# arjunchandra/paac

Hardware: AMD Instinct MI355X
Metric: global env-steps/sec at 32 envs, t_max=5, Nature net; 1/2/4/8 MI355X (higher is better)
Workload: dtype f32; 1 GPU; breakout action set (A=4), NATURE net, 32 envs per GPU x 1 GPU, t_max=5, synthetic 84x84x4 u8 frames generated on device, sampler=numpy, hipGraph replay; envs_per_gpu=32, t_max=5, global_envs=32, parallelism=env-sharded dp1, no collective (one process)

## Files before the change

paac_amd/csrc/api.hip:

```cpp
#include <stdarg.h>
#include <stdlib.h>

#include <new>

#include "common.h"

namespace paac {

static thread_local char g_err[512] = "";
thread_local ProfEvents g_prof = {nullptr, nullptr, 0, 0};
paac_ctx* g_prof_ctx = nullptr;

void set_error(const char* fmt, ...) {
  va_list ap;
  va_start(ap, fmt);
  vsnprintf(g_err, sizeof(g_err), fmt, ap);
  va_end(ap);
}

ArchSpec arch_spec(int arch) {
  ArchSpec s;
  memset(&s, 0, sizeof(s));
  if (arch == PAAC_ARCH_NATURE) {
    s.nconv = 3;
// ... 131 lines not shown
  c->max_batch = cfg->max_batch;
  for (int o = 0; o < OP_COUNT; ++o)
    for (int k = 0; k < 3; ++k) c->tune[o][k] = Tune{-1, 0, -1};
  default_tuning(c);
  if (const char* ov = getenv("PAAC_TUNE_OVERRIDE")) {
    int op, cls, cf, ks, xc, used = 0;
    while (sscanf(ov, "%d:%d:%d:%d:%d%n", &op, &cls, &cf, &ks, &xc, &used) == 5) {
      if (op >= 0 && op < OP_COUNT && cls >= 0 && cls < 3) c->tune[op][cls] = Tune{cf, ks, xc};
      ov += used;
      if (*ov != ',') break;
      ++ov;
    }
  }
  const int64_t B = cfg->max_batch;
  const int A = cfg->num_actions;
  c->fc_splits_max = fc_splits_max();
  for (int w = 0; w < 2; ++w) {
    Workspace& W = c->ws[w];
    for (int i = 0; i < c->spec.nconv; ++i) {
      const ConvSpec& cs = c->spec.conv[i];
      PAAC_CHECK_HIP(hipMalloc(&W.act[i], (size_t)((B + 15) / 16 * 16) * cs.oh * cs.ow * cs.cout * sizeof(float)));
    }
    PAAC_CHECK_HIP(hipMalloc(&W.fc_slab, (size_t)c->fc_splits_max * B * c->spec.fc * sizeof(float)));
    PAAC_CHECK_HIP(hipMalloc(&W.h, (size_t)B * c->spec.fc * sizeof(float)));
    PAAC_CHECK_HIP(hipMalloc(&W.probs, (size_t)B * A * sizeof(float)));
    PAAC_CHECK_HIP(hipMalloc(&W.logits, (size_t)B * A * sizeof(float)));
    PAAC_CHECK_HIP(hipMalloc(&W.values, (size_t)B * sizeof(float)));
  }
  for (int i = 0; i < c->spec.nconv; ++i) {
    const ConvSpec& cs = c->spec.conv[i];
    PAAC_CHECK_HIP(hipMalloc(&c->dact[i], (size_t)B * cs.oh * cs.ow * cs.cout * sizeof(float)));
  }
  PAAC_CHECK_HIP(hipMalloc(&c->dh, (size_t)B * c->spec.fc * sizeof(float)));
  PAAC_CHECK_HIP(hipMalloc(&c->dl_buf, (size_t)B * paac::kDlStride * sizeof(float)));
  PAAC_CHECK_HIP(hipMalloc(&c->ppo_rows, (size_t)B * 2 * sizeof(float)));
  PAAC_CHECK_HIP(hipMalloc(&c->vclip_rows, (size_t)B * sizeof(float)));
  c->wslab_floats = wslab_floats_needed(cfg->arch);
  PAAC_CHECK_HIP(hipMalloc(&c->wslab, (size_t)c->wslab_floats * sizeof(float)));
  PAAC_CHECK_HIP(hipMalloc(&c->partials, 8192 * sizeof(float)));
  PAAC_CHECK_HIP(hipMemset(c->partials, 0, 8192 * sizeof(float)));
  PAAC_CHECK_HIP(hipMalloc(&c->zeros, (size_t)(c->spec.fc > 1024 ? c->spec.fc : 1024) * sizeof(float)));
  PAAC_CHECK_HIP(hipMemset(c->zeros, 0, (size_t)(c->spec.fc > 1024 ? c->spec.fc : 1024) * sizeof(float)));
  c->keep_row = -1;
  c->keep_h_only = 0;
  c->heads_pending_h = 0;
  PAAC_CHECK_HIP(hipMalloc(&c->mt_ahead, mt_ahead_bytes()));
  PAAC_CHECK_HIP(hipMemset(c->mt_ahead, 0, mt_ahead_bytes()));
  c->ahead_state = nullptr;
  c->ahead_D = 0;
  {
    const char* v = getenv("PAAC_TOWER");
    c->tower_on = (cfg->arch == PAAC_ARCH_NATURE) && !(v && *v && atoi(v) == 0);
    { const char* q = getenv("PAAC_FC_QUARTER"); c->no_quarter_tiles = (q && *q && atoi(q) == 0) ? 1 : 0; }
    c->tower2_on = (cfg->arch == PAAC_ARCH_NIPS) && tower2_available() && !(v && *v && atoi(v) == 0);
    c->managed_weights = 0;
    c->tower_pack = nullptr;
    if (c->tower_on || c->tower2_on) PAAC_CHECK_HIP(hipMalloc(&c->tower_pack, tower_pack_bytes()));
    PAAC_CHECK_HIP(hipMalloc(&c->fc_pack, (size_t)c->spec.flat * c->spec.fc * sizeof(float)));
  }
  c->ev_start = new hipEvent_t[paac_ctx::PROF_MAX_EVENTS];
  c->ev_stop = new hipEvent_t[paac_ctx::PROF_MAX_EVENTS];
  c->ev_family = new int[paac_ctx::PROF_MAX_EVENTS];
  c->ev_batch = new int[paac_ctx::PROF_MAX_EVENTS];
  c->ev_mix = new int[paac_ctx::PROF_MAX_EVENTS];
  c->ev_count = 0;
  c->prof_on = 0;
  for (int i = 0; i < paac_ctx::PROF_MAX_EVENTS; ++i) {
    c->ev_start[i] = nullptr;
    c->ev_stop[i] = nullptr;
  }
  *out = c;
  return 0;
}

int paac_destroy(paac_ctx* c) {
  if (!c) return 0;
  for (int w = 0; w < 2; ++w) {
    Workspace& W = c->ws[w];
    for (int i = 0; i < 3; ++i)
      if (W.act[i]) (void)hipFree(W.act[i]);
    float* bufs[] = {W.fc_slab, W.h, W.probs, W.logits, W.values};
    for (float* b : bufs)
      if (b) (void)hipFree(b);
  }
  for (int i = 0; i < 3; ++i)
    if (c->dact[i]) (void)hipFree(c->dact[i]);
  float* bufs[] = {c->dh, c->wslab, c->partials, c->dl_buf, c->zeros, c->ppo_rows, c->vclip_rows};
  for (float* b : bufs)
    if (b) (void)hipFree(b);
  if (c->mt_ahead) (void)hipFree(c->mt_ahead);
  if (c->tower_pack) (void)hipFree(c->tower_pack);
  if (c->fc_pack) (void)hipFree(c->fc_pack);
  for (int i = 0; i < paac_ctx::PROF_MAX_EVENTS; ++i) {
    if (c->ev_start[i]) (void)hipEventDestroy(c->ev_start[i]);
    if (c->ev_stop[i]) (void)hipEventDestroy(c->ev_stop[i]);
  }
  delete[] c->ev_start;
  delete[] c->ev_stop;
  delete[] c->ev_family;
  delete[] c->ev_batch;
  delete[] c->ev_mix;
  delete c;
  return 0;
}

int paac_forward(paac_ctx* ctx, const float* params, const uint8_t* states, int batch, float* logits, float* probs,
                 float* values, paac_stream_t stream) {
  PAAC_REQUIRE(ctx && params && states, "paac_forward: null argument");
  PAAC_REQUIRE(batch > 0 && batch <= ctx->max_batch, "paac_forward: batch %d outside (0, max_batch=%d]", batch,
               ctx->max_batch);
  const int rc = launch_forward(ctx, 0, params, states, batch, logits, probs, values, (hipStream_t)stream);
  if (rc) return rc;
  PAAC_CHECK_HIP(hipGetLastError());
  return 0;
}

int paac_pack_weights(paac_ctx* ctx, const float* params, paac_stream_t stream) {
  PAAC_REQUIRE(ctx && params, "paac_pack_weights: null argument");
  const int rc = launch_pack_weights(ctx, params, (hipStream_t)stream);
  if (rc) return rc;
  PAAC_CHECK_HIP(hipGetLastError());
  return 0;
}
// ... 555 lines not shown
```

paac_amd/csrc/common.h:

```cpp
#pragma once
#include <hip/hip_runtime.h>
#include <hip/hip_ext.h>
#include <stdint.h>
#include <stdio.h>
#include <string.h>

#include "../../include/paac_hip.h"

namespace paac {

void set_error(const char* fmt, ...);

#define PAAC_CHECK_HIP(expr)                                                              \
  do {                                                                                    \
    hipError_t _e = (expr);                                                               \
    if (_e != hipSuccess) {                                                               \
      paac::set_error("%s:%d: %s -> %s", __FILE__, __LINE__, #expr, hipGetErrorString(_e)); \
      return -2;                                                                          \
    }                                                                                     \
  } while (0)

#define PAAC_REQUIRE(cond, ...)          \
  do {                                   \
    if (!(cond)) {                       \
// ... 19 lines not shown
enum Family {
  F_CONV1_FWD = 0, F_CONV2_FWD, F_CONV3_FWD, F_FC_FWD, F_HEADS_FWD,
  F_HEADS_BWD, F_FC_WGRAD, F_FC_DGRAD, F_CONV3_WGRAD, F_CONV3_DGRAD, F_CONV2_WGRAD, F_CONV2_DGRAD, F_CONV1_WGRAD,
  F_GRAD_FINALIZE, F_CLIP_RMSPROP, F_MISC,
  F_ENV_STEP, F_SAMPLE_ENV_STEP, F_SAMPLE_MT, F_SAMPLE_PHILOX, F_NSTEP_RETURNS, F_PREPROCESS_STACK, F_CONV_TOWER,
  F_FC_CONV3_WGRAD, F_CONV2_CONV1_WGRAD, F_DGRAD_TOWER
};
static_assert(F_DGRAD_TOWER + 1 == PAAC_PROF_FAMILIES, "family count");

}

namespace paac {
struct Workspace {
  float* act[3];
  float* fc_slab;
  float* h;
  float* probs;
  float* values;
  float* logits;
};
}

namespace paac {
enum Op { OP_CONV1_FWD = 0, OP_CONV2_FWD, OP_CONV3_FWD, OP_FC_FWD, OP_FC_WGRAD, OP_FC_DGRAD, OP_CONV3_WGRAD,
          OP_CONV3_DGRAD, OP_CONV2_WGRAD, OP_CONV2_DGRAD, OP_CONV1_WGRAD, OP_CONV_TOWER, OP_COUNT };
struct Tune {
  int cfg;
  int ksplit;
  int xcd;
};
inline int batch_class(int batch) { return batch > 512 ? 2 : batch > 64 ? 1 : 0; }

constexpr int kDlStride = 36;

struct FinalizeSeg {
  const float* src;
  float* dst;
  int count;
  int splits;
  long stride;
};
struct FinalizeArgs {
  FinalizeSeg seg[8];
  int nseg;
};

}

struct paac_ctx {
  paac_cfg cfg;
  paac::Tune tune[paac::OP_COUNT][3];
  paac::ArchSpec spec;
  paac_layout layout;
  int max_batch;
  paac::Workspace ws[2];
  int last_ws;
  float* dact[3];
  float* dh;
  float* wslab;
  int64_t wslab_floats;
  float* partials;
  int last_clip_local;
  paac::FinalizeArgs pending_fin;
  const float* pending_fin_grad;
  int heads_pending_rows, heads_pending_splits;
  int keep_row;
  int keep_h_only;
  int heads_pending_h;
  float* zeros;
  void* mt_ahead;
  const uint32_t* ahead_state;
  int ahead_D;
  float* dl_buf;
  float* ppo_rows;
  float* vclip_rows;
  int fc_splits_max;
  void* tower_pack;
  void* fc_pack;
  int tower_on;
  int heads_ntiles;
  int no_quarter_tiles;
  int tower2_on;
  int managed_weights;
  int prof_on;
  static constexpr int PROF_MAX_EVENTS = 8192;
  hipEvent_t* ev_start;
  hipEvent_t* ev_stop;
  int* ev_family;
  int* ev_batch;
  int* ev_mix;
  int ev_count;
// ... 106 lines not shown
```

paac_amd/csrc/heads.h:

```cpp
#pragma once
#include "common.h"
#include "synth_dev.h"

namespace paac {

constexpr int FC_SPLITS_MAX = 8;
constexpr int MAXA = 32;

#ifdef PAAC_DMM_STAMPS
__device__ unsigned long long* g_stamps_dev = nullptr;
#define HEADS_STAMP_INIT() unsigned long long* stamp_ptr = g_stamps_dev
#define HEADS_STAMP(i)                                                                                         \
  do {                                                                                                         \
    __builtin_amdgcn_sched_barrier(0);                                                                         \
    if (stamp_ptr && threadIdx.x == 0) stamp_ptr[(long)blockIdx.x * 8 + (i)] = (unsigned long long)clock64(); \
    __builtin_amdgcn_sched_barrier(0);                                                                         \
  } while (0)
#else
#define HEADS_STAMP_INIT()
#define HEADS_STAMP(i)
#endif

template <int NV>
__device__ __forceinline__ void block_sums_256(const float (&vals)[NV], float* scratch, float* out_lds) {
  const int tid = threadIdx.x;
#pragma unroll
  for (int a = 0; a < NV; ++a) scratch[a * 256 + tid] = vals[a];
  __syncthreads();
  float* stage = scratch + NV * 256;
  for (int u = tid; u < NV * 8; u += 256) {
    const int a = u >> 3, c = u & 7;
    float v[32];
#pragma unroll
    for (int i = 0; i < 32; ++i) v[i] = scratch[a * 256 + c * 32 + ((i + c) & 31)];
// ... 409 lines not shown
    ceps = rt.ppo.clip_eps;
  }
  if constexpr (LOSS == kLossPpoVclip) {
    vold = rt.vc.v_old[i];
    veps = rt.vc.vclip_eps;
  }
  if (rt.v_boot) {
    returns_row(rt, i, yv, av);
  } else {
    yv = y[i];
    av = adv[i];
  }
  if (yv_out) {
    *yv_out = yv;
    *av_out = av;
  }
  if constexpr (LOSS == kLossPpoVclip)
    head_grad_row<AP, kLossPpoVclip>(pi, values[i], actions[i], yv, av, beta, s, A, out, stats, pold, ceps, pstats, vold, veps);
  else if constexpr (LOSS == kLossPpo)
    head_grad_row<AP, kLossPpo>(pi, values[i], actions[i], yv, av, beta, s, A, out, stats, pold, ceps, pstats);
  else
    head_grad_row<AP>(pi, values[i], actions[i], yv, av, beta, s, A, out, stats);
}

constexpr int HB_CHUNK = 256;
template <int H, int AP, int EST, int LOSS = kLossA3c>
__global__ __launch_bounds__(256) void heads_bwd_kernel(const float* __restrict__ probs, const float* __restrict__ values,
                                                        const int32_t* __restrict__ actions, const float* __restrict__ y,
                                                        const float* __restrict__ adv, const float* __restrict__ h,
                                                        const float* __restrict__ Wa, const float* __restrict__ Wc,
                                                        int A, int B, float beta, float* __restrict__ dH,
                                                        float* __restrict__ gWa, float* __restrict__ gba,
                                                        float* __restrict__ gWc, float* __restrict__ gbc,
                                                        float* __restrict__ loss_out,
                                                        const typename ArgsOf<EST, LOSS>::type rt) {
  constexpr int NV = AP + 1;
  constexpr int NS = NV + 3;
  const int tid = threadIdx.x;
  const float s = 5.0f / (float)B;
  HEADS_STAMP_INIT();
  HEADS_STAMP(0);
  __shared__ float smem[NS * 256 + NS * 8 > HB_CHUNK * NV ? NS * 256 + NS * 8 : HB_CHUNK * NV];
  __shared__ float red[NS];
  if ((int)blockIdx.x < B) {
    const int i = blockIdx.x;
    constexpr int JPT = H / 256;
    float hv[JPT], wcj[JPT], waj[JPT][AP];
#pragma unroll
    for (int jj = 0; jj < JPT; ++jj) {
      const int j = tid + jj * 256;
      hv[jj] = h[(long)i * H + j];
      wcj[jj] = Wc[j];
#pragma unroll
      for (int a = 0; a < AP; ++a) waj[jj][a] = Wa[j * A + (a < A ? a : 0)];
    }
    float dl[NV];
    load_row_and_grad<AP, LOSS>(probs, values, actions, y, adv, i, A, beta, s, dl, nullptr, rt);
#pragma unroll
    for (int jj = 0; jj < JPT; ++jj) {
      const int j = tid + jj * 256;
      float acc = dl[AP] * wcj[jj];
#pragma unroll
      for (int a = 0; a < AP; ++a) acc = fmaf(dl[a], waj[jj][a], acc);
      dH[(long)i * H + j] = hv[jj] > 0.f ? acc : 0.f;
    }
    HEADS_STAMP(1);
    return;
  }
  const int role = blockIdx.x - B;
  if (role < H / 32) {
    const int jj = tid & 31, ig = tid >> 5;
    const int j = role * 32 + jj;
    float acc[NV];
#pragma unroll
    for (int a = 0; a < NV; ++a) acc[a] = 0.f;
    for (int i0 = 0; i0 < B; i0 += HB_CHUNK) {
      const int cnt = min(HB_CHUNK, B - i0);
      float hv[HB_CHUNK / 8];
#pragma unroll
      for (int q = 0; q < HB_CHUNK / 8; ++q) {
        const int r = ig + 8 * q;
        hv[q] = h[(long)(i0 + (r < cnt ? r : 0)) * H + j];
      }
      __syncthreads();
      if (tid < cnt) {
        float dl[NV];
        load_row_and_grad<AP, LOSS>(probs, values, actions, y, adv, i0 + tid, A, beta, s, dl, nullptr, rt);
#pragma unroll
        for (int a = 0; a < NV; ++a) smem[tid * NV + a] = dl[a];
      }
      __syncthreads();
#pragma unroll
      for (int q = 0; q < HB_CHUNK / 8; ++q) {
        const int r = ig + 8 * q;
        if (r < cnt) {
#pragma unroll
          for (int a = 0; a < NV; ++a) acc[a] = fmaf(hv[q], smem[r * NV + a], acc[a]);
        }
// ... 46 lines not shown
      const int64_t step = *rt.global_step + rt.step_inc;
      *rt.global_step = step;
      double lr = 0.0;
      if (step <= rt.anneal) lr = rt.lr0 - ((double)step * rt.lr0 / (double)rt.anneal);
      *rt.lr_out = (float)lr;
    }
    if (rt.tick) *rt.tick += rt.tick_inc;
  }
  block_sums_256<NS>(accv, smem, red);
  if (tid < A) gba[tid] = red[tid];
  if (tid == AP) gbc[0] = red[AP];
  if (tid == 0 && loss_out) {
    const float actor = red[NV] / (float)B;
    const float critic = red[NV + 1] / (float)B;
    loss_out[0] = 5.0f * (actor + critic);
    loss_out[1] = actor;
    loss_out[2] = critic;
    loss_out[3] = red[NV + 2] / (float)B;
  }
  HEADS_STAMP(4);
}

static_assert(kDlStride == MAXA + 1 + 3, "floats per row in the dl buffer: AP + 1 gradients (padded to 33) + 3 loss terms");

template <int H, int AP, int EST, int LOSS = kLossA3c>
__global__ __launch_bounds__(256) void heads_train_kernel(const float* __restrict__ slab, int splits, long slab_stride,
                                                          const float* __restrict__ fc_b, const float* __restrict__ Wa,
                                                          const float* __restrict__ ba, const float* __restrict__ Wc,
                                                          const float* __restrict__ bc, int A, int B,
                                                          float* __restrict__ h_out, float* __restrict__ logits_ws,
                                                          float* __restrict__ probs_ws, float* __restrict__ values_ws,
                                                          const int32_t* __restrict__ actions, const float* __restrict__ y,
                                                          const float* __restrict__ adv, float beta, float* __restrict__ dH,
                                                          float* __restrict__ dl_buf,
                                                          const typename ArgsOf<EST, LOSS>::type rt) {
  constexpr int JPT = H / 256;
  constexpr int NV = AP + 1;
  constexpr int NB = NV + 1;
  const int i = blockIdx.x;
  const int tid = threadIdx.x;
  const bool boot = rt.boot_in_fwd != 0;
  const int ib = boot ? B + i % rt.N : i;
  const float head_bias = (tid < A) ? ba[tid] : ((tid == AP || tid == NV) ? bc[0] : 0.f);
  float sv[JPT][FC_SPLITS_MAX], sb[JPT][FC_SPLITS_MAX], bj[JPT], wcj[JPT], waj[JPT][AP];
#pragma unroll
  for (int jj = 0; jj < JPT; ++jj) {
    const int j = tid + jj * 256;
    if (splits == 1) {
      sv[jj][0] = slab[(long)i * H + j];
      sb[jj][0] = slab[(long)ib * H + j];
#pragma unroll
      for (int sp = 1; sp < FC_SPLITS_MAX; ++sp) sv[jj][sp] = sb[jj][sp] = 0.f;
    } else {
#pragma unroll
      for (int sp = 0; sp < FC_SPLITS_MAX; ++sp) {
        sv[jj][sp] = slab[(sp < splits ? sp : 0) * slab_stride + (long)i * H + j];
        sb[jj][sp] = slab[(sp < splits ? sp : 0) * slab_stride + (long)ib * H + j];
      }
    }
    bj[jj] = fc_b[j];
    wcj[jj] = Wc[j];
#pragma unroll
    for (int a = 0; a < AP; ++a) waj[jj][a] = Wa[j * A + (a < A ? a : 0)];
  }
  const int act = actions[i];
  float pold = 0.f, ypre = 0.f, apre = 0.f;
  if constexpr (loss_is_ppo(LOSS)) {
    pold = rt.ppo.p_old[i];
    ypre = y[i];
    apre = adv[i];
  }
  float vold = 0.f;
  if constexpr (LOSS == kLossPpoVclip) vold = rt.vc.v_old[i];
  typename PreOf<EST>::type npre;
  if (rt.rewards) npre = returns_preload(rt, i);
  float part[NB], hv[JPT];
#pragma unroll
  for (int a = 0; a < NB; ++a) part[a] = 0.f;
#pragma unroll
  for (int jj = 0; jj < JPT; ++jj) {
    const int j = tid + jj * 256;
    float s = 0.f, sbt = 0.f;
#pragma unroll
    for (int sp = 0; sp < FC_SPLITS_MAX; ++sp) {
      s += (sp < splits) ? sv[jj][sp] : 0.f;
      sbt += (sp < splits) ? sb[jj][sp] : 0.f;
    }
    s = fmaxf(s + bj[jj], 0.f);
    sbt = fmaxf(sbt + bj[jj], 0.f);
    hv[jj] = s;
    h_out[(long)i * H + j] = s;
#pragma unroll
    for (int a = 0; a < AP; ++a) part[a] = (a < A) ? fmaf(s, waj[jj][a], part[a]) : part[a];
    part[AP] = fmaf(s, wcj[jj], part[AP]);
    part[NV] = fmaf(sbt, wcj[jj], part[NV]);
  }
  __shared__ float scratch[NB * 256 + NB * 8];
  __shared__ float lg[NB];
  __shared__ float row_s[AP + 3];
  block_sums_256<NB>(part, scratch, lg);
  if (tid < NB) lg[tid] += head_bias;
  __syncthreads();
  if (tid == 0) {
    float m = lg[0];
#pragma unroll
    for (int a = 1; a < AP; ++a) m = (a < A) ? fmaxf(m, lg[a]) : m;
    float e[AP];
    float sum = 0.f;
#pragma unroll
    for (int a = 0; a < AP; ++a) {
      e[a] = (a < A) ? expf(lg[a] - m) : 0.f;
      sum += e[a];
    }
#pragma unroll
    for (int a = 0; a < AP; ++a) {
      const float pa = (a < A) ? e[a] / sum : 0.f;
      row_s[a] = pa;
      if (a < A) {
        probs_ws[(long)i * A + a] = pa;
        logits_ws[(long)i * A + a] = lg[a];
        if constexpr (LOSS == kLossA3cRecord) {
          if (a == act) rt.ppo.p_old[i] = pa;
        }
      }
    }
    values_ws[i] = lg[AP];
    float yv, av;
    if constexpr (loss_is_ppo(LOSS)) {
      yv = ypre;
      av = apre;
// ... 25 lines not shown
  for (int a = 0; a < AP; ++a) pi[a] = row_s[a];
  if constexpr (LOSS == kLossPpoVclip) {
    float pst[3];
    head_grad_row<AP, kLossPpoVclip>(pi, lg[AP], act, row_s[AP], row_s[AP + 1], beta, 5.0f / (float)B, A, dl, stats, pold,
                                     rt.ppo.clip_eps, pst, vold, rt.vc.vclip_eps);
    if (tid == 0) {
      rt.ppo.stat_rows[2 * i] = pst[0];
      rt.ppo.stat_rows[2 * i + 1] = pst[1];
      rt.vc.stat_rows[i] = pst[2];
    }
  } else if constexpr (LOSS == kLossPpo) {
    float pst[2];
    head_grad_row<AP, kLossPpo>(pi, lg[AP], act, row_s[AP], row_s[AP + 1], beta, 5.0f / (float)B, A, dl, stats, pold,
                                rt.ppo.clip_eps, pst);
    if (tid == 0) {
      rt.ppo.stat_rows[2 * i] = pst[0];
      rt.ppo.stat_rows[2 * i + 1] = pst[1];
    }
  } else {
    head_grad_row<AP>(pi, lg[AP], act, row_s[AP], row_s[AP + 1], beta, 5.0f / (float)B, A, dl, stats);
  }
  if (tid == 0) {
#pragma unroll
    for (int a = 0; a < NV; ++a) dl_buf[(long)i * kDlStride + a] = dl[a];
#pragma unroll
    for (int k = 0; k < 3; ++k) dl_buf[(long)i * kDlStride + MAXA + 1 + k] = stats[k];
  }
#pragma unroll
  for (int jj = 0; jj < JPT; ++jj) {
    const int j = tid + jj * 256;
    float acc = dl[AP] * wcj[jj];
#pragma unroll
    for (int a = 0; a < AP; ++a) acc = fmaf(dl[a], waj[jj][a], acc);
    dH[(long)i * H + j] = hv[jj] > 0.f ? acc : 0.f;
  }
}

template <int H, int AP>
__device__ __forceinline__ void heads_param_grads(const int role, const float* __restrict__ h,
                                                  const float* __restrict__ dl_buf, const int A, const int B,
                                                  float* __restrict__ gWa, float* __restrict__ gba, float* __restrict__ gWc,
                                                  float* __restrict__ gbc, float* __restrict__ loss_out, float* smem) {
  constexpr int NV = AP + 1;
  constexpr int NS = NV + 3;
  const int tid = threadIdx.x;
  if (role < H / 32) {
    const int jj = tid & 31, ig = tid >> 5;
    const int j = role * 32 + jj;
    float acc[NV];
#pragma unroll
    for (int a = 0; a < NV; ++a) acc[a] = 0.f;
    for (int i0 = 0; i0 < B; i0 += HB_CHUNK) {
      const int cnt = min(HB_CHUNK, B - i0);
      float hv[HB_CHUNK / 8];
#pragma unroll
      for (int q = 0; q < HB_CHUNK / 8; ++q) {
        const int r = ig + 8 * q;
        hv[q] = h[(long)(i0 + (r < cnt ? r : 0)) * H + j];
      }
      __syncthreads();
      if (tid < cnt) {
#pragma unroll
        for (int a = 0; a < NV; ++a) smem[tid * NV + a] = dl_buf[(long)(i0 + tid) * kDlStride + a];
      }
      __syncthreads();
#pragma unroll
      for (int q = 0; q < HB_CHUNK / 8; ++q) {
        const int r = ig + 8 * q;
// ... 74 lines not shown
```

paac_amd/csrc/net_bwd.hip:

```cpp
#include <type_traits>

#include "net_common.h"
#include "dgrad_tower.h"
#include "gemm3.h"

namespace paac {

template <int NDIM>
struct DgradN {
  static constexpr int TN = (NDIM % 64 == 0) ? 4 : (NDIM % 32 == 0) ? 2 : 1;
};
template <class G, int NDIM, int BCO, int EPI, int TM, int NWM, int WK, int PF, int XB = 0>
using DgradBody = Dmm<G, false, FRAG_K, FRAG_K, TM, DgradN<NDIM>::TN, NWM, 1, WK, BCO, EPI, false, PF, XB>;

template <int NDIM, int EPI>
static void resolve_dgrad(const GemmArgs& g, int zdim, Tune t, int& cfg, int& xcd) {
  constexpr int TN = DgradN<NDIM>::TN;
  cfg = t.cfg;
  xcd = t.xcd;
  if (cfg < 0) {
    const long tiles = (long)((g.M + 31) / 32) * ((g.N + 16 * TN - 1) / (16 * TN)) * zdim;
    cfg = (tiles <= 384) ? 1 : (tiles <= 1536) ? 2 : 3;
    xcd = (EPI == EPI_MASK_PARITY) ? 0 : -1;
  }
}

template <class G, int NDIM, int BCO, int EPI>
static void launch_dgrad(const GemmArgs& g, int zdim, Tune t, hipStream_t s) {
  int cfg, xcd;
  resolve_dgrad<NDIM, EPI>(g, zdim, t, cfg, xcd);
  if (cfg >= kSplitBf16) {
    switch (cfg - kSplitBf16) {
#define X(id, TM, NWM, WK, PF) \
  case id: launch_dmm<DgradBody<G, NDIM, BCO, EPI, TM, NWM, WK, split_pf(PF), 2>>(g, zdim, 1, xcd, s); return;
      PAAC_DGRAD_SPLIT_CFGS(X)
#undef X
// ... 222 lines not shown
                         const float* y, const float* adv, int batch, float beta, float* grad, float* loss_out,
                         int phase, const GaeArgs& rt, int estimator, int loss, const PpoArgs& ppo, const VclipArgs& vc,
                         float* ppo_stats_out, hipStream_t s) {
  const paac_layout& L = ctx->layout;
  Workspace& W = ctx->ws[1];
  const int cls = batch_class(batch);
  const int A = ctx->cfg.num_actions;
  const int i_w1 = 0, i_w2 = 2, i_w3 = 4;
  const int i_wf = (NT::NCONV == 3) ? 6 : 4;
  const int i_wa = i_wf + 2, i_wc = i_wf + 4;
  const float* wa = params + L.offset[i_wa];
  const float* wc = params + L.offset[i_wc];
  const float* wf = params + L.offset[i_wf];
  const float* w2 = params + L.offset[i_w2];
  const float* w3 = (NT::NCONV == 3) ? params + L.offset[i_w3] : nullptr;

  const bool do_fc = phase == 0 || phase == 1 || phase == 3, do_conv = phase == 0 || phase == 2 || phase == 3;
  bool fused_heads = false;
  if (ctx->heads_pending_rows > 0) {
    const bool boot_ok = !rt.boot_in_fwd || ctx->heads_pending_rows >= batch + rt.N;
    if (NT::NCONV == 3 && ctx->tower_on && (phase == 0 || phase == 3) && ctx->heads_pending_rows >= batch && boot_ok) {
      fused_heads = true;
    } else {
      const int rc = launch_deferred_heads(ctx, params, s);
      if (rc) return rc;
    }
  }
  GaeArgs rtl = rt;
  const ReturnsArgs& rtn = rtl;
  if (rtl.boot_in_fwd && !fused_heads) {
    rtl.v_boot = W.values + batch;
    rtl.boot_in_fwd = 0;
  }
  if (do_fc && fused_heads) {
    ProfScope ps(ctx, F_HEADS_BWD, batch, s);
    const int rows = ctx->heads_pending_rows;
    const float* fc_b = ctx->heads_pending_h ? (const float*)ctx->zeros : params + L.offset[i_wf + 1];
    if (loss != kLossA3c) {
      auto go = [&](auto est, auto lossc, const auto& ra) {
        launch_heads_train<NT::H, decltype(est)::value, decltype(lossc)::value>(
            A, dim3(batch), s, (const float*)W.fc_slab, ctx->heads_pending_splits, (long)rows * NT::H, fc_b, wa,
            params + L.offset[i_wa + 1], wc, params + L.offset[i_wc + 1], A, batch, W.h, W.logits, W.probs, W.values, actions, y,
            adv, beta, ctx->dh, ctx->dl_buf, ra);
      };
      launch_ppo_heads(go, loss, estimator, rtl, ppo, vc);
    } else if (estimator == kEstGae)
      launch_heads_train<NT::H, kEstGae>(A, dim3(batch), s, (const float*)W.fc_slab, ctx->heads_pending_splits, (long)rows * NT::H,
                                         fc_b, wa, params + L.offset[i_wa + 1], wc, params + L.offset[i_wc + 1], A,
                                         batch, W.h, W.logits, W.probs, W.values, actions, y, adv, beta, ctx->dh, ctx->dl_buf, rtl);
    else
      launch_heads_train<NT::H, kEstNstep>(A, dim3(batch), s, (const float*)W.fc_slab, ctx->heads_pending_splits, (long)rows * NT::H,
                                           fc_b, wa, params + L.offset[i_wa + 1], wc, params + L.offset[i_wc + 1], A,
                                           batch, W.h, W.logits, W.probs, W.values, actions, y, adv, beta, ctx->dh, ctx->dl_buf, rtn);
    ctx->heads_pending_rows = 0;
    ctx->heads_pending_h = 0;
  } else if (do_fc) {
    ProfScope ps(ctx, F_HEADS_BWD, batch, s);
    if (loss != kLossA3c) {
      auto go = [&](auto est, auto lossc, const auto& ra) {
        launch_heads_bwd<NT::H, decltype(est)::value, decltype(lossc)::value>(
            A, dim3(batch + NT::H / 32 + 1), s, (const float*)W.probs, (const float*)W.values, actions, y, adv, (const float*)W.h,
            wa, wc, A, batch, beta, ctx->dh, grad + L.offset[i_wa], grad + L.offset[i_wa + 1], grad + L.offset[i_wc],
            grad + L.offset[i_wc + 1], loss_out, ra);
      };
      launch_ppo_heads(go, loss, estimator, rtl, ppo, vc);
    } else if (estimator == kEstGae)
      launch_heads_bwd<NT::H, kEstGae>(A, dim3(batch + NT::H / 32 + 1), s, (const float*)W.probs, (const float*)W.values, actions, y,
                                       adv, (const float*)W.h, wa, wc, A, batch, beta, ctx->dh, grad + L.offset[i_wa],
                                       grad + L.offset[i_wa + 1], grad + L.offset[i_wc], grad + L.offset[i_wc + 1], loss_out, rtl);
    else
      launch_heads_bwd<NT::H, kEstNstep>(A, dim3(batch + NT::H / 32 + 1), s, (const float*)W.probs, (const float*)W.values, actions, y,
                                         adv, (const float*)W.h, wa, wc, A, batch, beta, ctx->dh, grad + L.offset[i_wa],
                                         grad + L.offset[i_wa + 1], grad + L.offset[i_wc], grad + L.offset[i_wc + 1], loss_out, rtn);
  }
  if (do_fc && loss == kLossPpo && ppo_stats_out)
    launch_k(ppo_stats_kernel, dim3(1), dim3(256), s, PROF_NONE, (const float*)ppo.stat_rows, batch, ppo_stats_out);
  if (do_fc && loss == kLossPpoVclip && ppo_stats_out)
    launch_k(ppo_vclip_stats_kernel, dim3(1), dim3(256), s, PROF_NONE, (const float*)ppo.stat_rows,
             (const float*)vc.stat_rows, batch, ppo_stats_out);
  const float* xf = (NT::NCONV == 3) ? W.act[2] : W.act[1];
  float* dxf = (NT::NCONV == 3) ? ctx->dact[2] : ctx->dact[1];
  FinalizeArgs fin;
  memset(&fin, 0, sizeof(fin));
  float* slab = ctx->wslab;
  int conv1_splits_done = 0;
  bool fc_wgrad_held = false;
  GemmArgs held_gw;
  int held_ks = 1, held_xcd = -1;
  memset(&held_gw, 0, sizeof(held_gw));
  auto wgrad_out = [&](int i_w, int feats, int cout, float* base, int splits) {
    const long stride = (long)(feats + 1) * cout;
    fin.seg[fin.nseg++] = FinalizeSeg{base, grad + L.offset[i_w], feats * cout, splits, stride};
    fin.seg[fin.nseg++] = FinalizeSeg{base + (long)feats * cout, grad + L.offset[i_w + 1], cout, splits, stride};
  };
  if (do_fc) {
    GemmArgs gw = make_args(xf, (size_t)batch * NT::FLAT * 4, ctx->dh, (size_t)batch * NT::H * 4, grad + L.offset[i_wf], nullptr, NT::FLAT, NT::H, batch, NT::H, NT::H);
    gw.slab_rows = NT::FLAT + 1;
    GemmArgs gd = make_args(ctx->dh, (size_t)batch * NT::H * 4, wf, (size_t)NT::FLAT * NT::H * 4, dxf, xf, batch, NT::FLAT, NT::H, 0, NT::FLAT);
    if constexpr (NT::NCONV == 3) {
      static const bool pair2 = env_int("PAAC_WGRAD_PAIR", 1) != 0;
      int wcfg, wks, wxcd;
      resolve_wgrad<false, NT::H>(gw, 1, ctx->tune[OP_FC_WGRAD][cls], wcfg, wks, wxcd);
      static const int gemm3_rows = env_int("PAAC_GEMM3_MIN_ROWS", 513);
      fc_wgrad_held = pair2 && do_conv && ctx->tower_on && wcfg == 1 && !(batch >= gemm3_rows && (batch % 32) == 0);
      held_gw = gw;
      held_ks = wks;
// ... 6 lines not shown
      memset(&a, 0, sizeof(a));
      a.A = xf; a.lda = NT::FLAT;
      a.B = ctx->dh; a.ldb = NT::H;
      a.out = grad + L.offset[i_wf]; a.ldo = NT::H;
      a.colsum_out = grad + L.offset[i_wf + 1];
      a.M = NT::FLAT; a.N = NT::H; a.K = batch;
      using D = Gemm3<false, false, EPI_SLAB, 4, 2, 2, 2>;
      a.MB = (NT::FLAT + D::TM - 1) / D::TM;
      a.NB = (NT::H + D::TN - 1) / D::TN;
      a.S = 1;
      a.stages_per_split = batch / 32;
      prof_mix(6);
      launch_k(gemm3_kernel<D>, dim3((unsigned)(a.MB * a.NB)), dim3(D::THREADS), s, PROF_WHOLE, a);
    } else if (!fc_wgrad_held) {
      ProfScope ps(ctx, F_FC_WGRAD, batch, s);
      launch_wgrad<typename NT::GFC, false, NT::H>(gw, 1, ctx->tune[OP_FC_WGRAD][cls], s);
    }
    ProfScope ps(ctx, F_FC_DGRAD, batch, s);
    if (batch >= gemm3_min_rows && (NT::H % 32) == 0) {
      Gemm3Args a;
      memset(&a, 0, sizeof(a));
      a.A = ctx->dh; a.lda = NT::H;
      a.B = wf; a.ldb = NT::H;
      a.out = dxf; a.ldo = NT::FLAT;
      a.mask = xf;
      a.M = batch; a.N = NT::FLAT; a.K = NT::H;
      using D = Gemm3<true, true, EPI_MASK>;
      a.MB = (batch + D::TM - 1) / D::TM;
      a.NB = (NT::FLAT + D::TN - 1) / D::TN;
      a.S = 1;
      a.stages_per_split = NT::H / 32;
      prof_mix(6);
      launch_k(gemm3_kernel<D>, dim3((unsigned)(a.MB * a.NB)), dim3(D::THREADS), s, PROF_WHOLE, a);
    } else {
      launch_dgrad<typename NT::GFCH, NT::FLAT, NT::H, EPI_MASK>(gd, 1, ctx->tune[OP_FC_DGRAD][cls], s);
    }
  }
  if (!do_conv) return 0;
  if constexpr (NT::NCONV == 3) {
    const int feats = NT::G3::FEATS;
    constexpr int P2 = NT::G2::OPIX, P3 = NT::G3::OPIX;
    GemmArgs gw = make_args(W.act[1], (size_t)batch * P2 * NT::C2 * 4, ctx->dact[2], (size_t)batch * P3 * NT::C3 * 4, slab, nullptr, feats, NT::C3, batch * P3, NT::C3, NT::C3);
    gw.slab_rows = feats + 1;
    GemmArgs gd = make_args(ctx->dact[2], (size_t)batch * P3 * NT::C3 * 4, w3, (size_t)feats * NT::C3 * 4, ctx->dact[1], W.act[1], batch * P2, NT::C2, 9 * NT::C3, 0, NT::C2);
    gd.tap_base[0] = 8 * NT::C2 * NT::C3;
    gd.tap_sh = -3 * NT::C2 * NT::C3;
    gd.tap_sw = -NT::C2 * NT::C3;
    int splits;
    int c3 = -1, k3 = 1, x3 = -1;
    resolve_wgrad<false, NT::C3>(gw, W_SPLITS_MAX, ctx->tune[OP_CONV3_WGRAD][cls], c3, k3, x3);
    if (fc_wgrad_held && c3 != 1) {
      ProfScope ps(ctx, F_FC_WGRAD, batch, s);
      launch_wgrad<typename NT::GFC, false, NT::H>(held_gw, 1, ctx->tune[OP_FC_WGRAD][cls], s);
      fc_wgrad_held = false;
    }
    if (fc_wgrad_held) {
      using DF = WgradBody<typename NT::GFC, false, NT::H, 4, 2, 2>;
      using D3 = WgradBody<typename NT::G3, false, NT::C3, 4, 2, 2>;
      PairArgs pa;
      pa.g0 = held_gw;
      pa.g1 = gw;
      ProfScope ps(ctx, F_FC_CONV3_WGRAD, batch, s);
      pa.count0 = (int)prepare_dmm<DF>(pa.g0, held_ks, held_ks, held_xcd);
      const int n1 = (int)prepare_dmm<D3>(pa.g1, k3, k3, x3);
      pa.first1 = (pa.count0 + 7) / 8 * 8;
      launch_k(dmm_pair_kernel<DF, D3>, dim3((unsigned)(pa.first1 + n1)), dim3(128), s, PROF_WHOLE, pa);
// ... 196 lines not shown
```

Baseline: 730,300 env-steps/s.

## Add single-pass FC dgrad kernel fed by bf16x3 dh planes written in heads

The heads backward kernels now also write dH as three bf16 planes (split3) in an MFMA-ready tiled layout. A new FC dgrad kernel reads those planes once, packs weight slices into LDS as bf16x3, and runs 16x16x32 bf16 MFMAs with a prefetch ring plus a ReLU-mask epilogue. This replaces the tuned generic dgrad GEMM for small batches (<=192 rows) and removes its separate operand conversion and split-K passes. The cost is extra plane stores and a syncthreads in the heads kernel, and a bf16x3 emulation of fp32 accuracy.

```diff
diff --git a/paac_amd/csrc/api.hip b/paac_amd/csrc/api.hip
--- a/paac_amd/csrc/api.hip
+++ b/paac_amd/csrc/api.hip
@@ -187,6 +187,11 @@
     PAAC_CHECK_HIP(hipMalloc(&c->dact[i], (size_t)B * cs.oh * cs.ow * cs.cout * sizeof(float)));
   }
   PAAC_CHECK_HIP(hipMalloc(&c->dh, (size_t)B * c->spec.fc * sizeof(float)));
+  if (paac::dh_planes_supported(c->spec.fc)) {
+    PAAC_CHECK_HIP(hipMalloc(&c->dh_planes, paac::dh_planes_bytes((int)B, c->spec.fc)));
+    PAAC_CHECK_HIP(hipMemset(c->dh_planes, 0, paac::dh_planes_bytes((int)B, c->spec.fc)));
+  }
+  { const char* v = getenv("PAAC_FC_DGRAD_ONCE"); c->fc_dgrad_once = !(v && *v && atoi(v) == 0); }
   PAAC_CHECK_HIP(hipMalloc(&c->dl_buf, (size_t)B * paac::kDlStride * sizeof(float)));
   PAAC_CHECK_HIP(hipMalloc(&c->ppo_rows, (size_t)B * 2 * sizeof(float)));
   PAAC_CHECK_HIP(hipMalloc(&c->vclip_rows, (size_t)B * sizeof(float)));
@@ -244,6 +249,7 @@
   for (float* b : bufs)
     if (b) (void)hipFree(b);
   if (c->mt_ahead) (void)hipFree(c->mt_ahead);
+  if (c->dh_planes) (void)hipFree(c->dh_planes);
   if (c->tower_pack) (void)hipFree(c->tower_pack);
   if (c->fc_pack) (void)hipFree(c->fc_pack);
   for (int i = 0; i < paac_ctx::PROF_MAX_EVENTS; ++i) {
diff --git a/paac_amd/csrc/common.h b/paac_amd/csrc/common.h
--- a/paac_amd/csrc/common.h
+++ b/paac_amd/csrc/common.h
@@ -75,6 +75,9 @@
 inline int batch_class(int batch) { return batch > 512 ? 2 : batch > 64 ? 1 : 0; }
 
 constexpr int kDlStride = 36;
+
+constexpr bool dh_planes_supported(int H) { return (H % 32) == 0 && H <= 1024; }
+inline size_t dh_planes_bytes(int max_batch, int H) { return (size_t)((max_batch + 15) / 16 * 16) * H * 6; }
 
 struct FinalizeSeg {
   const float* src;
@@ -100,6 +103,9 @@
   int last_ws;
   float* dact[3];
   float* dh;
+  void* dh_planes;
+  int dh_planes_rows;
+  int fc_dgrad_once;
   float* wslab;
   int64_t wslab_floats;
   float* partials;
diff --git a/paac_amd/csrc/fc_dgrad_once.h b/paac_amd/csrc/fc_dgrad_once.h
--- /dev/null
+++ b/paac_amd/csrc/fc_dgrad_once.h
@@ -0,0 +1,232 @@
+#pragma once
+#include "dmm.h"
+
+namespace paac {
+
+constexpr int kFcOnceWaves = 4;
+constexpr int kFcOnceTilesPerWave = 3;
+constexpr int kFcOnceMaxRows = 16 * kFcOnceWaves * kFcOnceTilesPerWave;
+constexpr int kFcOnceKParts = 4;
+
+template <int H>
+__device__ __forceinline__ void store_dh_planes(const float* row_lds, const int i, const int B, bf16x8* __restrict__ planes) {
+  if constexpr (dh_planes_supported(H)) {
+    if (!planes) return;
+    __syncthreads();
+    constexpr int KS = H / 32;
+    const int tid = threadIdx.x;
+    for (int k8 = tid; k8 < H / 8; k8 += 256) {
+      const int ks = k8 >> 2, kq = k8 & 3;
+      const f32x4 v0 = *reinterpret_cast<const f32x4*>(row_lds + 32 * ks + 4 * kq);
+      const f32x4 v1 = *reinterpret_cast<const f32x4*>(row_lds + 32 * ks + 16 + 4 * kq);
+      const float x[8] = {v0[0], v0[1], v0[2], v0[3], v1[0], v1[1], v1[2], v1[3]};
+      bf16x8 ph, pm, pl;
+      split3_bf16(x, ph, pm, pl);
+      bf16x8* dst = planes + ((long)((i >> 4) * KS + ks) * 3) * 64 + kq * 16;
+      dst[i & 15] = ph;
+      dst[64 + (i & 15)] = pm;
+      dst[128 + (i & 15)] = pl;
+      if (i == B - 1) {
+        const bf16x8 z = __builtin_bit_cast(bf16x8, (u32x4){0u, 0u, 0u, 0u});
+        for (int r = (i & 15) + 1; r < 16; ++r) {
+          dst[r] = z;
+          dst[64 + r] = z;
+          dst[128 + r] = z;
+        }
+      }
+    }
+  }
+}
+
+struct FcOnceArgs {
+  const void* planes;
+  unsigned planes_bytes;
+  const float* wf;
+  const float* xf;
+  float* dx;
+  int M, FLAT;
+#ifdef PAAC_DMM_STAMPS
+  unsigned long long* stamps;
+#endif
+};
+
+#ifdef PAAC_DMM_STAMPS
+#define FCONCE_STAMP(i)                                                                                      \
+  do {                                                                                                       \
+    __builtin_amdgcn_sched_barrier(0);                                                                       \
+    if (p.stamps && lane == 0)                                                                               \
+      p.stamps[((long)blockIdx.x * NW + wave) * 8 + (i)] =                                                   \
+          ((i) == 0 || (i) == 7) ? (unsigned long long)wall_clock64() : (unsigned long long)clock64();       \
+    __builtin_amdgcn_sched_barrier(0);                                                                       \
+  } while (0)
+#else
+#define FCONCE_STAMP(i)
+#endif
+
+template <int H, int CT, int NW, int TPW, int PF>
+struct FcOnce {
+  static constexpr int KS = H / 32;
+  static constexpr int THREADS = 64 * NW;
+  static constexpr int ITEMS = CT * KS * 64;
+  static constexpr int PASSES = ITEMS / THREADS;
+  static constexpr int RING = PF + 1;
+  static constexpr int GPP = (KS + kFcOnceKParts - 1) / kFcOnceKParts;
+  static constexpr int SMEM_BYTES = CT * 3 * KS * 64 * 16;
+  static_assert(ITEMS % THREADS == 0, "the weight slice divides over the threads");
+  static_assert(PF >= 1 && PF < KS, "prefetch depth");
+
+  template <int NT>
+  __device__ __forceinline__ static void tiles(const FcOnceArgs& p, const bf16x8* wl, const __amdgpu_buffer_rsrc_t rs,
+                                               const bf16x8 (&pre)[PF][TPW][3], const int rt0, const int n0, const int lane) {
+    const int li = lane & 15, q = lane >> 4;
+    bf16x8 fb[RING][NT][3];
+#pragma unroll
+    for (int s = 0; s < PF; ++s)
+#pragma unroll
+      for (int t = 0; t < NT; ++t)
+#pragma unroll
+        for (int pl = 0; pl < 3; ++pl) fb[s][t][pl] = pre[s][t][pl];
+    f32x4 mk[NT][CT];
+    int off[NT];
+#pragma unroll
+    for (int t = 0; t < NT; ++t) {
+      const int row = (rt0 + t * NW) * 16 + li;
+      off[t] = (row < p.M) ? row * p.FLAT + n0 + 4 * q : -1;
+#pragma unroll
+      for (int c = 0; c < CT; ++c)
+        mk[t][c] = (off[t] >= 0) ? *reinterpret_cast<const f32x4*>(p.xf + off[t] + 16 * c) : (f32x4){0.f, 0.f, 0.f, 0.f};
+    }
+    f32x4 acc[NT][CT], tot[NT][CT];
+#pragma unroll
+    for (int t = 0; t < NT; ++t)
+#pragma unroll
+      for (int c = 0; c < CT; ++c) acc[t][c] = tot[t][c] = (f32x4){0.f, 0.f, 0.f, 0.f};
+    bf16x8 wa[2][CT][3];
+#pragma unroll
+    for (int c = 0; c < CT; ++c)
+#pragma unroll
+      for (int pl = 0; pl < 3; ++pl) wa[0][c][pl] = wl[((c * 3 + pl) * KS + 0) * 64 + lane];
+#pragma unroll
+    for (int ks = 0; ks < KS; ++ks) {
+      if (ks + PF < KS) {
+#pragma unroll
+        for (int t = 0; t < NT; ++t)
+#pragma unroll
+          for (int pl = 0; pl < 3; ++pl)
+            fb[(ks + PF) % RING][t][pl] = __builtin_bit_cast(
+                bf16x8, __builtin_amdgcn_raw_buffer_load_b128(rs, (unsigned)lane * 16u,
+                                                              (unsigned)((((rt0 + t * NW) * KS + ks + PF) * 3 + pl) * 1024), 0));
+      }
+      if (ks + 1 < KS) {
+#pragma unroll
+        for (int c = 0; c < CT; ++c)
+#pragma unroll
+          for (int pl = 0; pl < 3; ++pl) wa[(ks + 1) & 1][c][pl] = wl[((c * 3 + pl) * KS + ks + 1) * 64 + lane];
+      }
+      __builtin_amdgcn_sched_barrier(0);
+      constexpr int PW[6] = {0, 1, 2, 0, 1, 0};
+      constexpr int PD[6] = {2, 1, 0, 1, 0, 0};
+#pragma unroll
+      for (int n = 0; n < 6; ++n)
+#pragma unroll
+        for (int t = 0; t < NT; ++t)
+#pragma unroll
+          for (int c = 0; c < CT; ++c)
+            acc[t][c] = __builtin_amdgcn_mfma_f32_16x16x32_bf16(wa[ks & 1][c][PW[n]], fb[ks % RING][t][PD[n]], acc[t][c], 0, 0, 0);
+      if ((ks + 1) % GPP == 0 || ks + 1 == KS) {
+#pragma unroll
+        for (int t = 0; t < NT; ++t)
+#pragma unroll
+          for (int c = 0; c < CT; ++c) {
+            tot[t][c] = (ks < GPP) ? acc[t][c] : tot[t][c] + acc[t][c];
+            acc[t][c] = (f32x4){0.f, 0.f, 0.f, 0.f};
+          }
+      }
+      __builtin_amdgcn_sched_barrier(0);
+    }
+#ifdef PAAC_DMM_STAMPS
+    const int wave = rt0;
+#endif
+    FCONCE_STAMP(4);
+    FCONCE_STAMP(5);
+#pragma unroll
+    for (int t = 0; t < NT; ++t) {
+      if (off[t] < 0) continue;
+#pragma unroll
+      for (int c = 0; c < CT; ++c) {
+        f32x4 v = tot[t][c];
+#pragma unroll
+        for (int e = 0; e < 4; ++e) v[e] = mk[t][c][e] > 0.f ? v[e] : 0.f;
+        *reinterpret_cast<f32x4*>(p.dx + off[t] + 16 * c) = v;
+      }
+    }
+  }
+
+  __device__ __forceinline__ static void run(const FcOnceArgs& p, char* smem) {
+    bf16x8* wl = reinterpret_cast<bf16x8*>(smem);
+    const int tid = threadIdx.x;
+    const int lane = tid & 63;
+    const int wave = __builtin_amdgcn_readfirstlane(tid >> 6);
+    const int n0 = blockIdx.x * (16 * CT);
+    const int ntiles = (p.M + 15) >> 4;
+    const int nt = (wave < ntiles) ? (ntiles - wave + NW - 1) / NW : 0;
+    const __amdgpu_buffer_rsrc_t rs = make_rsrc(p.planes, p.planes_bytes);
+    FCONCE_STAMP(0);
+    FCONCE_STAMP(1);
+    FCONCE_STAMP(2);
+    bf16x8 pre[PF][TPW][3];
+#pragma unroll
+    for (int s = 0; s < PF; ++s)
+#pragma unroll
+      for (int t = 0; t < TPW; ++t)
+#pragma unroll
+        for (int pl = 0; pl < 3; ++pl)
+          pre[s][t][pl] = __builtin_bit_cast(
+              bf16x8, __builtin_amdgcn_raw_buffer_load_b128(rs, (t < nt) ? (unsigned)lane * 16u : kOob,
+                                                            (unsigned)((((wave + t * NW) * KS + s) * 3 + pl) * 1024), 0));
+    f32x4 w0[PASSES], w1[PASSES];
+#pragma unroll
+    for (int ps = 0; ps < PASSES; ++ps) {
+      const int id = ps * THREADS + tid;
+      const int l = id & 63, ks = (id >> 6) % KS, c = id / (64 * KS);
+      const float* src = p.wf + (long)(n0 + 16 * c + (l & 15)) * H + 32 * ks + 4 * (l >> 4);
+      w0[ps] = *reinterpret_cast<const f32x4*>(src);
+      w1[ps] = *reinterpret_cast<const f32x4*>(src + 16);
+    }
+    __builtin_amdgcn_sched_barrier(0);
+#pragma unroll
+    for (int ps = 0; ps < PASSES; ++ps) {
+      const int id = ps * THREADS + tid;
+      const int l = id & 63, ks = (id >> 6) % KS, c = id / (64 * KS);
+      const float x[8] = {w0[ps][0], w0[ps][1], w0[ps][2], w0[ps][3], w1[ps][0], w1[ps][1], w1[ps][2], w1[ps][3]};
+      bf16x8 ph, pm, pl;
+      split3_bf16(x, ph, pm, pl);
+      wl[((c * 3 + 0) * KS + ks) * 64 + l] = ph;
+      wl[((c * 3 + 1) * KS + ks) * 64 + l] = pm;
+      wl[((c * 3 + 2) * KS + ks) * 64 + l] = pl;
+    }
+    __syncthreads();
+    FCONCE_STAMP(3);
+    if (nt == 0) {
+      FCONCE_STAMP(4);
+      FCONCE_STAMP(5);
+      FCONCE_STAMP(6);
+      FCONCE_STAMP(7);
+      return;
+    }
+    static_assert(TPW >= 1 && TPW <= 3, "row tiles per wave");
+    if (nt == 1) tiles<1>(p, wl, rs, pre, wave, n0, lane);
+    if constexpr (TPW >= 2) { if (nt == 2) tiles<2>(p, wl, rs, pre, wave, n0, lane); }
+    if constexpr (TPW >= 3) { if (nt >= 3) tiles<3>(p, wl, rs, pre, wave, n0, lane); }
+    FCONCE_STAMP(6);
+    FCONCE_STAMP(7);
+  }
+};
+
+template <class D>
+__global__ __launch_bounds__(D::THREADS) void fc_dgrad_once_kernel(const FcOnceArgs p) {
+  __shared__ __attribute__((aligned(16))) char smem[D::SMEM_BYTES];
+  D::run(p, smem);
+}
+
+}
diff --git a/paac_amd/csrc/heads.h b/paac_amd/csrc/heads.h
--- a/paac_amd/csrc/heads.h
+++ b/paac_amd/csrc/heads.h
@@ -1,5 +1,6 @@
 #pragma once
 #include "common.h"
+#include "fc_dgrad_once.h"
 #include "synth_dev.h"
 
 namespace paac {
@@ -475,7 +476,7 @@
                                                         int A, int B, float beta, float* __restrict__ dH,
                                                         float* __restrict__ gWa, float* __restrict__ gba,
                                                         float* __restrict__ gWc, float* __restrict__ gbc,
-                                                        float* __restrict__ loss_out,
+                                                        float* __restrict__ loss_out, bf16x8* __restrict__ dh_planes,
                                                         const typename ArgsOf<EST, LOSS>::type rt) {
   constexpr int NV = AP + 1;
   constexpr int NS = NV + 3;
@@ -483,7 +484,7 @@
   const float s = 5.0f / (float)B;
   HEADS_STAMP_INIT();
   HEADS_STAMP(0);
-  __shared__ float smem[NS * 256 + NS * 8 > HB_CHUNK * NV ? NS * 256 + NS * 8 : HB_CHUNK * NV];
+  __shared__ __attribute__((aligned(16))) float smem[NS * 256 + NS * 8 > HB_CHUNK * NV ? NS * 256 + NS * 8 : HB_CHUNK * NV];
   __shared__ float red[NS];
   if ((int)blockIdx.x < B) {
     const int i = blockIdx.x;
@@ -505,8 +506,11 @@
       float acc = dl[AP] * wcj[jj];
 #pragma unroll
       for (int a = 0; a < AP; ++a) acc = fmaf(dl[a], waj[jj][a], acc);
-      dH[(long)i * H + j] = hv[jj] > 0.f ? acc : 0.f;
-    }
+      const float d = hv[jj] > 0.f ? acc : 0.f;
+      dH[(long)i * H + j] = d;
+      if constexpr (dh_planes_supported(H)) smem[j] = d;
+    }
+    store_dh_planes<H>(smem, i, B, dh_planes);
     HEADS_STAMP(1);
     return;
   }
@@ -619,7 +623,7 @@
                                                           float* __restrict__ probs_ws, float* __restrict__ values_ws,
                                                           const int32_t* __restrict__ actions, const float* __restrict__ y,
                                                           const float* __restrict__ adv, float beta, float* __restrict__ dH,
-                                                          float* __restrict__ dl_buf,
+                                                          float* __restrict__ dl_buf, bf16x8* __restrict__ dh_planes,
                                                           const typename ArgsOf<EST, LOSS>::type rt) {
   constexpr int JPT = H / 256;
   constexpr int NV = AP + 1;
@@ -682,7 +686,7 @@
     part[AP] = fmaf(s, wcj[jj], part[AP]);
     part[NV] = fmaf(sbt, wcj[jj], part[NV]);
   }
-  __shared__ float scratch[NB * 256 + NB * 8];
+  __shared__ __attribute__((aligned(16))) float scratch[NB * 256 + NB * 8];
   __shared__ float lg[NB];
   __shared__ float row_s[AP + 3];
   block_sums_256<NB>(part, scratch, lg);
@@ -774,8 +778,11 @@
     float acc = dl[AP] * wcj[jj];
 #pragma unroll
     for (int a = 0; a < AP; ++a) acc = fmaf(dl[a], waj[jj][a], acc);
-    dH[(long)i * H + j] = hv[jj] > 0.f ? acc : 0.f;
-  }
+    const float d = hv[jj] > 0.f ? acc : 0.f;
+    dH[(long)i * H + j] = d;
+    if constexpr (dh_planes_supported(H)) scratch[j] = d;
+  }
+  store_dh_planes<H>(scratch, i, B, dh_planes);
 }
 
 template <int H, int AP>
diff --git a/paac_amd/csrc/net_bwd.hip b/paac_amd/csrc/net_bwd.hip
--- a/paac_amd/csrc/net_bwd.hip
+++ b/paac_amd/csrc/net_bwd.hip
@@ -2,6 +2,7 @@
 
 #include "net_common.h"
 #include "dgrad_tower.h"
+#include "fc_dgrad_once.h"
 #include "gemm3.h"
 
 namespace paac {
@@ -290,6 +291,11 @@
     rtl.v_boot = W.values + batch;
     rtl.boot_in_fwd = 0;
   }
+  static const int gemm3_rows_once = env_int("PAAC_GEMM3_MIN_ROWS", 513);
+  const bool once_shape = ctx->fc_dgrad_once && ctx->dh_planes && dh_planes_supported(NT::H) && batch <= kFcOnceMaxRows &&
+                          batch < gemm3_rows_once && (NT::FLAT % 16) == 0;
+  bf16x8* dhp = once_shape ? reinterpret_cast<bf16x8*>(ctx->dh_planes) : nullptr;
+  if (do_fc) ctx->dh_planes_rows = dhp ? batch : 0;
   if (do_fc && fused_heads) {
     ProfScope ps(ctx, F_HEADS_BWD, batch, s);
     const int rows = ctx->heads_pending_rows;
@@ -299,17 +305,17 @@
         launch_heads_train<NT::H, decltype(est)::value, decltype(lossc)::value>(
             A, dim3(batch), s, (const float*)W.fc_slab, ctx->heads_pending_splits, (long)rows * NT::H, fc_b, wa,
             params + L.offset[i_wa + 1], wc, params + L.offset[i_wc + 1], A, batch, W.h, W.logits, W.probs, W.values, actions, y,
-            adv, beta, ctx->dh, ctx->dl_buf, ra);
+            adv, beta, ctx->dh, ctx->dl_buf, dhp, ra);
       };
       launch_ppo_heads(go, loss, estimator, rtl, ppo, vc);
     } else if (estimator == kEstGae)
       launch_heads_train<NT::H, kEstGae>(A, dim3(batch), s, (const float*)W.fc_slab, ctx->heads_pending_splits, (long)rows * NT::H,
                                          fc_b, wa, params + L.offset[i_wa + 1], wc, params + L.offset[i_wc + 1], A,
-                                         batch, W.h, W.logits, W.probs, W.values, actions, y, adv, beta, ctx->dh, ctx->dl_buf, rtl);
+                                         batch, W.h, W.logits, W.probs, W.values, actions, y, adv, beta, ctx->dh, ctx->dl_buf, dhp, rtl);
     else
       launch_heads_train<NT::H, kEstNstep>(A, dim3(batch), s, (const float*)W.fc_slab, ctx->heads_pending_splits, (long)rows * NT::H,
                                            fc_b, wa, params + L.offset[i_wa + 1], wc, params + L.offset[i_wc + 1], A,
-                                           batch, W.h, W.logits, W.probs, W.values, actions, y, adv, beta, ctx->dh, ctx->dl_buf, rtn);
+                                           batch, W.h, W.logits, W.probs, W.values, actions, y, adv, beta, ctx->dh, ctx->dl_buf, dhp, rtn);
     ctx->heads_pending_rows = 0;
     ctx->heads_pending_h = 0;
   } else if (do_fc) {
@@ -319,17 +325,17 @@
         launch_heads_bwd<NT::H, decltype(est)::value, decltype(lossc)::value>(
             A, dim3(batch + NT::H / 32 + 1), s, (const float*)W.probs, (const float*)W.values, actions, y, adv, (const float*)W.h,
             wa, wc, A, batch, beta, ctx->dh, grad + L.offset[i_wa], grad + L.offset[i_wa + 1], grad + L.offset[i_wc],
-            grad + L.offset[i_wc + 1], loss_out, ra);
+            grad + L.offset[i_wc + 1], loss_out, dhp, ra);
       };
       launch_ppo_heads(go, loss, estimator, rtl, ppo, vc);
     } else if (estimator == kEstGae)
       launch_heads_bwd<NT::H, kEstGae>(A, dim3(batch + NT::H / 32 + 1), s, (const float*)W.probs, (const float*)W.values, actions, y,
                                        adv, (const float*)W.h, wa, wc, A, batch, beta, ctx->dh, grad + L.offset[i_wa],
-                                       grad + L.offset[i_wa + 1], grad + L.offset[i_wc], grad + L.offset[i_wc + 1], loss_out, rtl);
+                                       grad + L.offset[i_wa + 1], grad + L.offset[i_wc], grad + L.offset[i_wc + 1], loss_out, dhp, rtl);
     else
       launch_heads_bwd<NT::H, kEstNstep>(A, dim3(batch + NT::H / 32 + 1), s, (const float*)W.probs, (const float*)W.values, actions, y,
                                          adv, (const float*)W.h, wa, wc, A, batch, beta, ctx->dh, grad + L.offset[i_wa],
-                                         grad + L.offset[i_wa + 1], grad + L.offset[i_wc], grad + L.offset[i_wc + 1], loss_out, rtn);
+                                         grad + L.offset[i_wa + 1], grad + L.offset[i_wc], grad + L.offset[i_wc + 1], loss_out, dhp, rtn);
   }
   if (do_fc && loss == kLossPpo && ppo_stats_out)
     launch_k(ppo_stats_kernel, dim3(1), dim3(256), s, PROF_NONE, (const float*)ppo.stat_rows, batch, ppo_stats_out);
@@ -402,6 +408,23 @@
       a.stages_per_split = NT::H / 32;
       prof_mix(6);
       launch_k(gemm3_kernel<D>, dim3((unsigned)(a.MB * a.NB)), dim3(D::THREADS), s, PROF_WHOLE, a);
+    } else if (once_shape && ctx->dh_planes_rows == batch) {
+      if constexpr (dh_planes_supported(NT::H) && (NT::FLAT % 16) == 0) {
+        using D = FcOnce<NT::H, 1, kFcOnceWaves, kFcOnceTilesPerWave, 3>;
+        FcOnceArgs a;
+        a.planes = ctx->dh_planes;
+        a.planes_bytes = (unsigned)dh_planes_bytes(batch, NT::H);
+        a.wf = wf;
+        a.xf = xf;
+        a.dx = dxf;
+        a.M = batch;
+        a.FLAT = NT::FLAT;
+#ifdef PAAC_DMM_STAMPS
+        a.stamps = gd.stamps;
+#endif
+        prof_mix(6);
+        launch_k(fc_dgrad_once_kernel<D>, dim3(NT::FLAT / 16), dim3(D::THREADS), s, PROF_WHOLE, a);
+      }
     } else {
       launch_dgrad<typename NT::GFCH, NT::FLAT, NT::H, EPI_MASK>(gd, 1, ctx->tune[OP_FC_DGRAD][cls], s);
     }
```

New measurement: 737,900 env-steps/s, median of 6. 1.01x the previous value.
